# maybeLx/MVSFormerPlusPlus

Hardware: NVIDIA H100
Metric: depth-maps/sec (hot path: FMT + 4-stage cascade) (higher is better)
Workload: dtype f32

## Files before the change

mvsformerplusplus_b200/csrc/warp_corr.cu:

```cuda
#include <float.h>

#include <atomic>
#include <mutex>

#include "warp_geom.cuh"

namespace mvsf {

bool warp_tile_supported(const float* feat, int C, int G, int D, int H, int W);
int warp_tile_entropy(const float* feat, const float* homs, const float* depth, float* entropy, int V, int C, int D, int H,
                      int W, cudaStream_t s);
int warp_tile_aggregate(const float* feat, const float* homs, const float* depth, const float* vis, float* volume, int V, int C,
                        int D, int H, int W, cudaStream_t s);
bool warp_stream_store_supported(const float* feat, const float* corr, int C, int G, int D, int H, int W);
int warp_stream_entropy_store(const float* feat, const float* homs, const float* depth, float* entropy, float* corr, int V,
                              int H, int W, int* select, int max_miss_permille, cudaStream_t s);

constexpr int kMaxGenericD = 512;

template <int C>
struct WC {
  static constexpr int LPP = C / 4, P = 32 / LPP, DCH = 2 * LPP;
};
struct __align__(16) TapTable {
  int4 off[64];
  float4 wt[64];
};

template <int C>
__device__ __forceinline__ void build_taps(TapTable& tb, const float* __restrict__ depth, const Hom& m, const float3& ray,
                                           const CoordConst& cc, int p1, int d0, int D, int HW, int H, int W, int lane) {
  constexpr int P = WC<C>::P;
#pragma unroll
  for (int k = 0; k < 2; ++k) {
    const int t = lane + 32 * k;
    const int d = d0 + t / P;
    const float dv = (d < D) ? __ldg(depth + (size_t)d * HW + p1) : 1.0f;
    float ix, iy;
    warp_coord_fast(ray, m, dv, cc, ix, iy);
    int4 off;
    float4 wt;
    make_tap_fast(ix, iy, W, H, C, off, wt);
    tb.off[t] = off;
    tb.wt[t] = wt;
  }
}
__device__ __forceinline__ float4 gather4(const float* __restrict__ base, const int4& o, const float4& w) {
  float4 a = ldg4(base + o.x), b = ldg4(base + o.y), c = ldg4(base + o.z), d = ldg4(base + o.w);
  float4 s;
// ... 83 lines not shown
      }
    }
    __syncwarp();
    ReduceScatter<DCH, LPP>::run(part, lip);
#pragma unroll
    for (int i = 0; i < SPL; ++i) {
      const int d = d0 + lip * SPL + i;
      sims[ch * SPL + i] = (d < D) ? part[i] * gscale : -FLT_MAX;
    }
  }
  float mx = -FLT_MAX;
  for (int i = 0; i < nch * SPL; ++i) mx = fmaxf(mx, sims[i]);
#pragma unroll
  for (int o = LPP / 2; o > 0; o >>= 1) mx = fmaxf(mx, __shfl_xor_sync(0xffffffffu, mx, o));
  float Z = 0.f;
  for (int i = 0; i < nch * SPL; ++i) {
    sims[i] = (sims[i] == -FLT_MAX) ? 0.f : expf(sims[i] - mx);
    Z += sims[i];
  }
#pragma unroll
  for (int o = LPP / 2; o > 0; o >>= 1) Z += __shfl_xor_sync(0xffffffffu, Z, o);
  float ent = 0.f;
  for (int i = 0; i < nch * SPL; ++i) {
    float pr = __fdiv_rn(sims[i], Z);
    ent -= pr * logf(pr + 1e-7f);
  }
#pragma unroll
  for (int o = LPP / 2; o > 0; o >>= 1) ent += __shfl_xor_sync(0xffffffffu, ent, o);
  if (active && lip == 0) entropy[(size_t)v * HW + p2] = ent;
  if (STRIDED) __syncwarp();
  } while (STRIDED && (bx += (int)gridDim.x) * 8 * P < HW);
}

template <int C, int CPG>
__global__ void __launch_bounds__(256)
warp_corr_aggregate_kernel(const float* __restrict__ feat, const float* __restrict__ homs,
                           const float* __restrict__ depth, const float* __restrict__ vis,
                           float* __restrict__ volume, int V, int D, int H, int W) {
  constexpr int LPP = WC<C>::LPP, P = WC<C>::P, DCH = WC<C>::DCH;
  constexpr int G = C / CPG;
  constexpr int NGL = (CPG >= 4) ? 1 : 4 / CPG;
  constexpr int LPG = (CPG >= 4) ? CPG / 4 : 1;
  static_assert(LPG == 1 || LPG == 2, "C/G must be 1, 2, 4 or 8");
  __shared__ TapTable tables[8];
  const int lane = threadIdx.x & 31, warp = threadIdx.x >> 5;
  TapTable& tb = tables[warp];
  const int HW = H * W;
  const int pix0 = (blockIdx.x * 8 + warp) * P;
  if (pix0 >= HW) return;
  const int p1 = min(pix0 + lane % P, HW - 1);
  const int p2raw = pix0 + lane / LPP;
  const bool active = p2raw < HW;
  const int p2 = active ? p2raw : HW - 1;
  const int lip = lane % LPP, pi = lane / LPP;
  const CoordConst cc = make_coord_const(W, H);
  const int y1 = p1 / W, x1 = p1 - y1 * W;
  const float fx = (float)x1, fy = (float)y1;
  const float4 r = ldg4(feat + (size_t)p2 * C + lip * 4);
  constexpr float inv_cpg = 1.0f / (float)CPG;

  for (int d0 = 0; d0 < D; d0 += DCH) {
    float acc[NGL][DCH];
#pragma unroll
    for (int g = 0; g < NGL; ++g)
#pragma unroll
      for (int i = 0; i < DCH; ++i) acc[g][i] = 0.f;
    float wsum = 0.f;
    for (int v = 0; v < V - 1; ++v) {
      const Hom m = load_hom(homs + (size_t)v * 12);
      const float3 ray = ref_ray(m, fx, fy);
      build_taps<C>(tb, depth, m, ray, cc, p1, d0, D, HW, H, W, lane);
      __syncwarp();
      const float* __restrict__ src = feat + (size_t)(v + 1) * HW * C + lip * 4;
      const float w = __ldg(vis + (size_t)v * HW + p2);
      wsum = __fadd_rn(wsum, w);
#pragma unroll
      for (int di = 0; di < DCH; ++di) {
        const int4 o = tb.off[di * P + pi];
        const float4 wt = tb.wt[di * P + pi];
        const float4 s = gather4(src, o, wt);
        if (CPG >= 4) {
// ... 8 lines not shown
          acc[NGL > 2 ? 2 : 0][di] = fmaf(r.z * s.z, w, acc[NGL > 2 ? 2 : 0][di]);
          acc[NGL > 3 ? 3 : 0][di] = fmaf(r.w * s.w, w, acc[NGL > 3 ? 3 : 0][di]);
        }
      }
      __syncwarp();
    }
    const float den = __fadd_rn(wsum, 1e-6f);
    if (LPG == 2) {
      ReduceScatter<DCH, 2>::run(acc[0], lip & 1);
      if (active) {
        const int dbase = d0 + (lip & 1) * (DCH / 2);
#pragma unroll
        for (int i = 0; i < DCH / 2; ++i)
          if (dbase + i < D) volume[((size_t)(dbase + i) * HW + p2) * G + (lip >> 1)] = __fdiv_rn(acc[0][i], den);
      }
    } else if (active) {
#pragma unroll
      for (int di = 0; di < DCH; ++di) {
        if (d0 + di < D) {
          float* o = volume + ((size_t)(d0 + di) * HW + p2) * G;
          if (NGL == 1) {
            o[lip] = __fdiv_rn(acc[0][di], den);
          } else if (NGL == 2) {
            *reinterpret_cast<float2*>(o + lip * 2) = make_float2(__fdiv_rn(acc[0][di], den), __fdiv_rn(acc[NGL > 1 ? 1 : 0][di], den));
          } else {
            *reinterpret_cast<float4*>(o + lip * 4) =
                make_float4(__fdiv_rn(acc[0][di], den), __fdiv_rn(acc[NGL > 1 ? 1 : 0][di], den),
                            __fdiv_rn(acc[NGL > 2 ? 2 : 0][di], den), __fdiv_rn(acc[NGL > 3 ? 3 : 0][di], den));
          }
        }
      }
    }
  }
}

__global__ void homo_warp_kernel(const float* __restrict__ src, const float* __restrict__ hom,
                                 const float* __restrict__ depth, float* __restrict__ warped,
                                 uint8_t* __restrict__ mask, int C, int D, int H, int W) {
  const int HW = H * W;
  int p = blockIdx.x * blockDim.x + threadIdx.x;
  int d = blockIdx.y;
  if (p >= HW) return;
  int y = p / W, x = p - y * W;
  const Hom m = load_hom(hom);
  const float3 ray = ref_ray(m, (float)x, (float)y);
  const float half_w = (float)(W - 1) * 0.5f, half_h = (float)(H - 1) * 0.5f;
  float ix, iy, z;
  warp_coord(ray, m, __ldg(depth + (size_t)d * HW + p), half_w, half_h, (float)(W - 1), (float)(H - 1), ix, iy, z);
  Tap t = make_tap(ix, iy, W, H, C);
  for (int c = 0; c < C; ++c) {
    float a = __ldg(src + t.o00 + c), b = __ldg(src + t.o01 + c), cc = __ldg(src + t.o10 + c), dd = __ldg(src + t.o11 + c);
    warped[((size_t)c * D + d) * HW + p] = fmaf(dd, t.w11, fmaf(cc, t.w10, fmaf(b, t.w01, a * t.w00)));
  }
  if (mask) {
    bool out = (ix > (float)(W - 1)) || (ix < 0.0f) || (iy > (float)(H - 1)) || (iy < 0.0f) || (z <= 0.0f);
    mask[(size_t)d * HW + p] = out ? 1 : 0;
  }
}

template <int C>
static void launch_entropy(const float* feat, const float* homs, const float* depth, float* entropy, float* corr, int V, int G,
                           int D, int H, int W, cudaStream_t s) {
  constexpr int P = WC<C>::P;
  dim3 grid(cdiv((long long)H * W, 8 * P), V - 1);
  if (corr) {
    if (D == WC<C>::DCH)
      warp_corr_entropy_kernel<C, false, C / 8><<<grid, 256, 0, s>>>(feat, homs, depth, entropy, corr, G, D, H, W, nullptr);
    else
      warp_corr_entropy_kernel<C, true, C / 8><<<grid, 256, 0, s>>>(feat, homs, depth, entropy, corr, G, D, H, W, nullptr);
  } else if (D == WC<C>::DCH) {
    warp_corr_entropy_kernel<C, false, 0><<<grid, 256, 0, s>>>(feat, homs, depth, entropy, nullptr, G, D, H, W, nullptr);
  } else {
    warp_corr_entropy_kernel<C, true, 0><<<grid, 256, 0, s>>>(feat, homs, depth, entropy, nullptr, G, D, H, W, nullptr);
  }
}

static void launch_entropy_behind_select(const float* feat, const float* homs, const float* depth, float* entropy, float* corr,
                                         int V, int H, int W, cudaStream_t s, const int* skip_if) {
  constexpr int P = WC<8>::P;
  dim3 grid(cdiv((long long)H * W, 8 * P), V - 1);
  const int cap = device_sm_count(current_device()) * 16;
  if ((int)grid.x > cap) grid.x = cap;
  warp_corr_entropy_kernel<8, false, 1, true><<<grid, 256, 0, s>>>(feat, homs, depth, entropy, corr, 8, WC<8>::DCH, H, W, skip_if);
}

__global__ void __launch_bounds__(256)
corr_aggregate_kernel(const float* __restrict__ corr, const float* __restrict__ vis, float* __restrict__ volume, int V, int D,
                      int HW) {
  const size_t i = (size_t)blockIdx.x * blockDim.x + threadIdx.x;
  const size_t total = (size_t)D * HW * 2;
  if (i >= total) return;
  const size_t dp = i >> 1;
  const int p = (int)(dp % HW);
  float4 acc = make_float4(0.f, 0.f, 0.f, 0.f);
  float wsum = 0.f;
  for (int v = 0; v < V - 1; ++v) {
    const float w = __ldg(vis + (size_t)v * HW + p);
    const float4 c = ldg4(corr + ((size_t)v * D * HW + dp) * 8 + (i & 1) * 4);
    wsum = __fadd_rn(wsum, w);
    acc.x = fmaf(c.x, w, acc.x); acc.y = fmaf(c.y, w, acc.y); acc.z = fmaf(c.z, w, acc.z); acc.w = fmaf(c.w, w, acc.w);
  }
  const float den = __fadd_rn(wsum, 1e-6f);
  *reinterpret_cast<float4*>(volume + dp * 8 + (i & 1) * 4) =
      make_float4(__fdiv_rn(acc.x, den), __fdiv_rn(acc.y, den), __fdiv_rn(acc.z, den), __fdiv_rn(acc.w, den));
}

template <int C, int CPG>
static int launch_aggregate(const float* feat, const float* homs, const float* depth, const float* vis, float* volume,
                            int V, int D, int H, int W, cudaStream_t s) {
  constexpr int P = WC<C>::P;
  dim3 grid(cdiv((long long)H * W, 8 * P));
  warp_corr_aggregate_kernel<C, CPG><<<grid, 256, 0, s>>>(feat, homs, depth, vis, volume, V, D, H, W);
  return 0;
}

}

using namespace mvsf;

static int g_use_tile = 1;
constexpr int kMaxMissPermille = 60;

constexpr int kSelectSlots = 256;
static int* g_select[16] = {};
static std::atomic<unsigned> g_select_next{0};
static std::atomic<int*> g_select_last{nullptr};
static std::mutex g_select_mu;
static int* select_slot() {
  const int dev = current_device();
  if (dev < 0 || dev >= 16) return nullptr;
  if (!g_select[dev]) {
    std::lock_guard<std::mutex> lock(g_select_mu);
    if (!g_select[dev]) {
      int* p = nullptr;
      if (cudaMalloc(&p, sizeof(int) * 8 * kSelectSlots) != cudaSuccess) return nullptr;
      cudaMemset(p, 0, sizeof(int) * 8 * kSelectSlots);
      g_select[dev] = p;
    }
  }
  int* slot = g_select[dev] + 8 * (g_select_next.fetch_add(1) % kSelectSlots);
  g_select_last.store(slot);
  return slot;
}

extern "C" {
// ... 18 lines not shown
int mvsf_warp_corr_plan(int C, int G, int D, int H, int W, int V, size_t spill_budget_bytes) {
  if (G != 8 || !(C == 8 || C == 16 || C == 32 || C == 64)) return 1;
  const size_t spill = (size_t)4 * (size_t)(V > 1 ? V - 1 : 1) * G * D * H * W;
  return spill > spill_budget_bytes ? 1 : 0;
}
int mvsf_warp_corr_entropy(const float* feat, const float* homs, const float* depth, float* entropy, int V, int C,
                           int G, int D, int H, int W, mvsf_stream_t stream) {
  return warp_corr_entropy_impl(feat, homs, depth, entropy, nullptr, V, C, G, D, H, W, stream);
}

int mvsf_warp_corr_entropy_store(const float* feat, const float* homs, const float* depth, float* entropy, float* corr,
                                 int V, int C, int G, int D, int H, int W, mvsf_stream_t stream) {
  MVSF_REQUIRE(corr && ((uintptr_t)corr & 15) == 0 && G == 8, "warp_corr_entropy_store: corr must be 16-byte aligned and G == 8");
  return warp_corr_entropy_impl(feat, homs, depth, entropy, corr, V, C, G, D, H, W, stream);
}

int mvsf_corr_aggregate(const float* corr, const float* vis, float* volume, int V, int G, int D, int H, int W,
                        mvsf_stream_t stream) {
  MVSF_REQUIRE(corr && vis && volume && V >= 2 && G == 8 && D >= 1 && H > 0 && W > 0, "corr_aggregate: bad arguments (G must be 8)");
  const size_t total = (size_t)D * H * W * 2;
  corr_aggregate_kernel<<<cdiv((long long)total, 256), 256, 0, (cudaStream_t)stream>>>(corr, vis, volume, V, D, H * W);
  MVSF_LAUNCH_CHECK("corr_aggregate");
  return MVSF_OK;
}

static int warp_corr_entropy_impl(const float* feat, const float* homs, const float* depth, float* entropy, float* corr, int V,
                                  int C, int G, int D, int H, int W, mvsf_stream_t stream) {
  MVSF_REQUIRE(feat && homs && depth && entropy, "warp_corr_entropy: null pointer");
  MVSF_REQUIRE(V >= 2 && H > 0 && W > 0 && D >= 1, "warp_corr_entropy: bad shape");
  MVSF_REQUIRE(G <= C, "G must <= C!");
  MVSF_REQUIRE(C % G == 0 && (C == 8 || C == 16 || C == 32 || C == 64), "warp_corr_entropy: C must be 8/16/32/64, C %% G == 0");
  MVSF_REQUIRE(D <= kMaxGenericD, "warp_corr_entropy: D <= %d", kMaxGenericD);
  cudaStream_t s = (cudaStream_t)stream;
  const bool pipeline = corr && g_use_tile && warp_stream_store_supported(feat, corr, C, G, D, H, W);
  if (pipeline && g_use_tile == 2) {
    int rc = warp_stream_entropy_store(feat, homs, depth, entropy, corr, V, H, W, nullptr, kMaxMissPermille, s);
    if (rc) return rc;
    MVSF_LAUNCH_CHECK("warp_stream_entropy_store");
    return MVSF_OK;
  }
  int* select = pipeline ? select_slot() : nullptr;
  if (select) {
    int rc = warp_stream_entropy_store(feat, homs, depth, entropy, corr, V, H, W, select, kMaxMissPermille, s);
    if (rc) return rc;
    count_launch();
    MVSF_LAUNCH_CHECK("warp_stream_entropy_store");
    launch_entropy_behind_select(feat, homs, depth, entropy, corr, V, H, W, s, select);
    MVSF_LAUNCH_CHECK("warp_corr_entropy");
    return MVSF_OK;
  }
  if (!corr && g_use_tile && warp_tile_supported(feat, C, G, D, H, W)) {
    int rc = warp_tile_entropy(feat, homs, depth, entropy, V, C, D, H, W, s);
    if (rc) return rc;
    MVSF_LAUNCH_CHECK("warp_tile_entropy");
    return MVSF_OK;
  }
  switch (C) {
    case 8: launch_entropy<8>(feat, homs, depth, entropy, corr, V, G, D, H, W, s); break;
    case 16: launch_entropy<16>(feat, homs, depth, entropy, corr, V, G, D, H, W, s); break;
    case 32: launch_entropy<32>(feat, homs, depth, entropy, corr, V, G, D, H, W, s); break;
    default: launch_entropy<64>(feat, homs, depth, entropy, corr, V, G, D, H, W, s); break;
  }
  MVSF_LAUNCH_CHECK("warp_corr_entropy");
  return MVSF_OK;
}

int mvsf_warp_corr_aggregate(const float* feat, const float* homs, const float* depth, const float* vis,
                             float* volume, int V, int C, int G, int D, int H, int W, mvsf_stream_t stream) {
  MVSF_REQUIRE(feat && homs && depth && vis && volume, "warp_corr_aggregate: null pointer");
  MVSF_REQUIRE(V >= 2 && H > 0 && W > 0 && D >= 1, "warp_corr_aggregate: bad shape");
  MVSF_REQUIRE(G <= C, "G must <= C!");
  MVSF_REQUIRE(G == 8 && (C == 8 || C == 16 || C == 32 || C == 64), "warp_corr_aggregate: G must be 8 and C in 8/16/32/64");
  cudaStream_t s = (cudaStream_t)stream;
  if (g_use_tile && warp_tile_supported(feat, C, G, D, H, W)) {
    int rc = warp_tile_aggregate(feat, homs, depth, vis, volume, V, C, D, H, W, s);
    if (rc) return rc;
    MVSF_LAUNCH_CHECK("warp_tile_aggregate");
    return MVSF_OK;
  }
  switch (C) {
    case 8: launch_aggregate<8, 1>(feat, homs, depth, vis, volume, V, D, H, W, s); break;
    case 16: launch_aggregate<16, 2>(feat, homs, depth, vis, volume, V, D, H, W, s); break;
    case 32: launch_aggregate<32, 4>(feat, homs, depth, vis, volume, V, D, H, W, s); break;
    default: launch_aggregate<64, 8>(feat, homs, depth, vis, volume, V, D, H, W, s); break;
  }
  MVSF_LAUNCH_CHECK("warp_corr_aggregate");
  return MVSF_OK;
}

int mvsf_homo_warp(const float* src_nhwc, const float* hom, const float* depth, float* warped, uint8_t* mask, int C,
                   int D, int H, int W, mvsf_stream_t stream) {
  MVSF_REQUIRE(src_nhwc && hom && depth && warped && C > 0 && D > 0 && H > 0 && W > 0 && D <= 65535, "homo_warp: bad arguments");
  dim3 grid(cdiv(H * W, 128), D);
  homo_warp_kernel<<<grid, 128, 0, (cudaStream_t)stream>>>(src_nhwc, hom, depth, warped, mask, C, D, H, W);
  MVSF_LAUNCH_CHECK("homo_warp");
  return MVSF_OK;
}
}
```

mvsformerplusplus_b200/csrc/warp_tile.cu:

```cuda
#include <float.h>
#include <limits.h>

#include "warp_geom.cuh"
#include "wgmma.cuh"

namespace mvsf {
namespace wt {
using namespace gmma;

constexpr int TW = 32, THREADS = 256;
constexpr int kMaxD = 512;
constexpr int kPassBBlocks8 = 3;
constexpr int kPsBlocks = 2, kPsNbuf = 3;

template <int C>
struct Cfg {
  static constexpr int LPX = C / 8;
  static constexpr int PIX = THREADS / LPX;
  static constexpr int TROWS = PIX / TW;
  static constexpr int WX = 64, WY = 16;
  static constexpr int POS = 2 * C * 4;
  static constexpr int P = WX * POS;
  static constexpr uint32_t BYTES = (WY / 2) * P;
};

__device__ __forceinline__ void mbar_wait_warp(uint32_t bar, uint32_t parity) {
  if ((threadIdx.x & 31) == 0) {
    uint32_t it = 0;
    while (!mbar_try_wait(bar, parity))
      if (++it > (1u << MVSF_MBAR_SPIN_LOG2)) __trap();
  }
  __syncwarp();
}
__device__ __forceinline__ float4 lds128(uint32_t addr) {
  float4 v;
  asm volatile("ld.shared.v4.f32 {%0, %1, %2, %3}, [%4];" : "=f"(v.x), "=f"(v.y), "=f"(v.z), "=f"(v.w) : "r"(addr));
  return v;
}
__device__ __forceinline__ void fma4(float4& acc, float w, const float4& t) {
  acc = make_float4(fmaf(t.x, w, acc.x), fmaf(t.y, w, acc.y), fmaf(t.z, w, acc.z), fmaf(t.w, w, acc.w));
}
__device__ __forceinline__ float dot4(const float4& a, const float4& b) { return fmaf(a.w, b.w, fmaf(a.z, b.z, fmaf(a.y, b.y, a.x * b.x))); }

struct Lane {
  bool b0, b1, b2;
  uint32_t base[2];
};
template <int C>
__device__ __forceinline__ Lane make_lane(int lane, int sub, uint32_t win, int& chA, int& chB) {
  Lane L;
  if (C == 8) {
    L.b0 = lane & 1; L.b1 = (lane >> 1) & 1; L.b2 = (lane >> 2) & 1;
    L.base[0] = win + (L.b0 ? 16 : 0);
    L.base[1] = win + (L.b0 ? 0 : 16);
    chA = L.b0 ? 4 : 0; chB = L.b0 ? 0 : 4;
  } else {
    L.b0 = false; L.b1 = (lane >> 1) & 1; L.b2 = (lane >> 2) & 1;
    const int q0 = 2 * sub + (L.b1 ? 1 : 0), q1 = 2 * sub + (L.b1 ? 0 : 1);
    L.base[0] = win + q0 * 16;
    L.base[1] = win + q1 * 16;
    chA = q0 * 4; chB = q1 * 4;
  }
  return L;
}

template <int C>
__device__ __forceinline__ void gather_window(const Lane& L, int lx, int ly, float fx, float fy, float4& sA, float4& sB) {
  using K = Cfg<C>;
  const float gx = 1.0f - fx, gy = 1.0f - fy;
  const bool yodd = ly & 1;
// ... 243 lines not shown
      for (int k = 0; k < DCHT; ++k) accA[k] = accB[k] = make_float4(0.f, 0.f, 0.f, 0.f);
      for (int v = 0; v < V - 1; ++v) {
        const ViewCtx<C> vc = make_view(v);
        const float w = __ldg(vis + (size_t)v * HW + p);
        process_chunk<C, DCHT>(&map, sh, win, slot, phase, L, vc, v + 1, depth_p, HW, d0, n, active, cc, W, H,
                               [&](int k, const float4& sA, const float4& sB) {
                                 accA[k].x = fmaf(qA.x * sA.x, w, accA[k].x); accA[k].y = fmaf(qA.y * sA.y, w, accA[k].y);
                                 accA[k].z = fmaf(qA.z * sA.z, w, accA[k].z); accA[k].w = fmaf(qA.w * sA.w, w, accA[k].w);
                                 accB[k].x = fmaf(qB.x * sB.x, w, accB[k].x); accB[k].y = fmaf(qB.y * sB.y, w, accB[k].y);
                                 accB[k].z = fmaf(qB.z * sB.z, w, accB[k].z); accB[k].w = fmaf(qB.w * sB.w, w, accB[k].w);
                               });
      }
      if (active) {
#pragma unroll
        for (int k = 0; k < DCHT; ++k) {
          if (k < n) {
            float* o = out + ((size_t)(d0 + k) * HW + p) * 8;
            if (C == 8) {
              *reinterpret_cast<float4*>(o + chA) = make_float4(__fdiv_rn(accA[k].x, den), __fdiv_rn(accA[k].y, den),
                                                                __fdiv_rn(accA[k].z, den), __fdiv_rn(accA[k].w, den));
              *reinterpret_cast<float4*>(o + chB) = make_float4(__fdiv_rn(accB[k].x, den), __fdiv_rn(accB[k].y, den),
                                                                __fdiv_rn(accB[k].z, den), __fdiv_rn(accB[k].w, den));
            } else {
              *reinterpret_cast<float2*>(o + chA / 2) = make_float2(__fdiv_rn(accA[k].x + accA[k].y, den), __fdiv_rn(accA[k].z + accA[k].w, den));
              *reinterpret_cast<float2*>(o + chB / 2) = make_float2(__fdiv_rn(accB[k].x + accB[k].y, den), __fdiv_rn(accB[k].z + accB[k].w, den));
            }
          }
        }
      }
    }
  }
}

template <int C>
struct PsCfg {
  static constexpr int NCONS = 256 * Cfg<C>::LPX;
  static constexpr int THREADS = NCONS + 32;
  static constexpr int TROWS = 8;
};

template <int NBUF>
struct PsShared {
  unsigned long long full[NBUF], empty[NBUF];
  int origin[NBUF][2];
};

template <int C>
__device__ __forceinline__ int2 sample_pixel(int tile, int tiles_x, int lane, int W, int H) {
  const int sr = (lane >> 3) * 2 + 1, sc = (lane & 7) * 4 + 1;
  return make_int2(min((tile % tiles_x) * TW + sc, W - 1), min((tile / tiles_x) * PsCfg<C>::TROWS + sr, H - 1));
}
template <int C>
__device__ __forceinline__ int2 predict_window(const Hom& m, const float3& ray, float d_first, float d_last, const CoordConst& cc,
                                               int W, int H) {
  Bbox b;
#pragma unroll
  for (int e = 0; e < 2; ++e) {
    float ix, iy;
    warp_coord_lean(ray, m, e ? d_last : d_first, cc, ix, iy);
    b.add(split_coord(ix, iy, W, H));
  }
  b.reduce_warp();
  return window_origin<C>(b);
}

template <int C, int D, int NBUF>
__global__ void __launch_bounds__(PsCfg<C>::THREADS, kPsBlocks)
warp_stream_entropy_store_kernel(const __grid_constant__ CUtensorMap map, const float* __restrict__ feat,
                                 const float* __restrict__ homs, const float* __restrict__ depth, float* __restrict__ entropy,
                                 float* __restrict__ corr, int V, int H, int W, int tiles_x, int ntiles,
                                 const int* __restrict__ select) {
  using K = Cfg<C>;
  using P = PsCfg<C>;
  extern __shared__ __align__(128) unsigned char smem_raw[];
  __shared__ PsShared<NBUF> sh;
  if (select && *select == 0) return;
  const uint32_t win0 = (smem_u32(smem_raw) + 127u) & ~127u;
  const int tid = threadIdx.x, lane = tid & 31, warp = tid >> 5;
  const int HW = H * W;
  if (tid == 0) {
    for (int b = 0; b < NBUF; ++b) { mbar_init(smem_u32(&sh.full[b]), 1); mbar_init(smem_u32(&sh.empty[b]), P::NCONS / 32); }
    fence_barrier_init();
  }
  __syncthreads();
  const CoordConst cc = make_coord_const(W, H);
  const int my_tiles = (ntiles - (int)blockIdx.x + (int)gridDim.x - 1) / (int)gridDim.x;

  if (warp == P::NCONS / 32) {
    int j = 0;
    for (int t = 0; t < my_tiles; ++t) {
      const int2 sp = sample_pixel<C>((int)blockIdx.x + t * (int)gridDim.x, tiles_x, lane, W, H);
      const int p = sp.y * W + sp.x;
      const float d_first = __ldg(depth + p), d_last = __ldg(depth + (size_t)(D - 1) * HW + p);
      for (int v = 0; v < V - 1; ++v, ++j) {
        const int buf = j % NBUF;
        const Hom m = load_hom(homs + (size_t)v * 12);
        const int2 o = predict_window<C>(m, ref_ray(m, (float)sp.x, (float)sp.y), d_first, d_last, cc, W, H);
        mbar_wait_warp(smem_u32(&sh.empty[buf]), (uint32_t)(((j / NBUF) & 1) ^ 1));
        if (lane == 0) {
          sh.origin[buf][0] = o.x;
          sh.origin[buf][1] = o.y;
          const uint32_t bar = smem_u32(&sh.full[buf]);
          expect_tx(bar, K::BYTES);
          tma_load_5d(win0 + (uint32_t)buf * K::BYTES, &map, 0, 0, o.x, o.y >> 1, v + 1, bar);
        }
        __syncwarp();
      }
    }
    return;
  }

  const int pix_in_cta = tid / K::LPX, sub = tid % K::LPX;
  int chA, chB;
  const Lane L0 = make_lane<C>(lane, sub, 0u, chA, chB);
  constexpr float inv_cpg = 8.0f / (float)C;
  int j = 0;
  for (int t = 0; t < my_tiles; ++t) {
    const int tile = (int)blockIdx.x + t * (int)gridDim.x;
    const int px = (tile % tiles_x) * TW + (pix_in_cta % TW), py = (tile / tiles_x) * P::TROWS + (pix_in_cta / TW);
    const bool active = (px < W) && (py < H);
    const int p = min(py, H - 1) * W + min(px, W - 1);
    const float fxp = (float)min(px, W - 1), fyp = (float)min(py, H - 1);
    const float4 rA = ldg4(feat + (size_t)p * C + chA), rB = ldg4(feat + (size_t)p * C + chB);
    float dv[D];
#pragma unroll
    for (int k = 0; k < D; ++k) dv[k] = __ldg(depth + (size_t)k * HW + p);
    for (int v = 0; v < V - 1; ++v, ++j) {
      const int buf = j % NBUF;
      const Hom m = load_hom(homs + (size_t)v * 12);
      const float3 ray = ref_ray(m, fxp, fyp);
      const float* __restrict__ src = feat + (size_t)(v + 1) * HW * C;
      mbar_wait_warp(smem_u32(&sh.full[buf]), (uint32_t)((j / NBUF) & 1));
      const int ox = sh.origin[buf][0], oy = sh.origin[buf][1];
      const uint32_t wbuf = win0 + (uint32_t)buf * K::BYTES;
      const Lane L = {L0.b0, L0.b1, L0.b2, {wbuf + L0.base[0], wbuf + L0.base[1]}};
      float sims[D];
      float mx = -FLT_MAX;
#pragma unroll
      for (int k = 0; k < D; ++k) {
        float ix, iy;
        warp_coord_lean(ray, m, dv[k], cc, ix, iy);
        TapCoord tc = split_coord(ix, iy, W, H);
        tc.inb = tc.inb && active;
        float4 sA = make_float4(0.f, 0.f, 0.f, 0.f), sB = sA;
        const int lx = tc.x0 - ox, ly = tc.y0 - oy;
        const bool inwin = in_window<C>(tc.inb, lx, ly);
        gather_window<C>(L, inwin ? lx : 0, inwin ? ly : 0, tc.fx, tc.fy, sA, sB);
        if (!inwin) {
          sA = make_float4(0.f, 0.f, 0.f, 0.f); sB = sA;
          if (tc.inb) gather_global<C>(src + chA, src + chB, ix, iy, W, H, sA, sB);
        }
        if (active) {
          float* cp = corr + (((size_t)v * D + k) * HW + p) * 8;
          if (C == 8) {
            *reinterpret_cast<float4*>(cp + chA) = make_float4(rA.x * sA.x, rA.y * sA.y, rA.z * sA.z, rA.w * sA.w);
            *reinterpret_cast<float4*>(cp + chB) = make_float4(rB.x * sB.x, rB.y * sB.y, rB.z * sB.z, rB.w * sB.w);
          } else {
            *reinterpret_cast<float2*>(cp + chA / 2) = make_float2(fmaf(rA.y, sA.y, rA.x * sA.x) * inv_cpg, fmaf(rA.w, sA.w, rA.z * sA.z) * inv_cpg);
            *reinterpret_cast<float2*>(cp + chB / 2) = make_float2(fmaf(rB.y, sB.y, rB.x * sB.x) * inv_cpg, fmaf(rB.w, sB.w, rB.z * sB.z) * inv_cpg);
          }
        }
        float s = dot4(rA, sA) + dot4(rB, sB);
        if (K::LPX == 2) s += __shfl_xor_sync(0xffffffffu, s, 1);
        s *= inv_cpg;
        sims[k] = s;
        mx = fmaxf(mx, s);
      }
      __syncwarp();
      if (lane == 0) mbar_arrive(smem_u32(&sh.empty[buf]));
      float Z = 0.f, ent = 0.f;
#pragma unroll
      for (int k = 0; k < D; ++k) { sims[k] = __expf(sims[k] - mx); Z += sims[k]; }
      const float rZ = __fdiv_rn(1.0f, Z);
#pragma unroll
      for (int k = 0; k < D; ++k) { const float pr = sims[k] * rZ; ent -= pr * __logf(pr + 1e-7f); }
      if (active && sub == 0) entropy[(size_t)v * HW + p] = ent;
    }
  }
}


template <int C, int D>
__global__ void __launch_bounds__(1024)
warp_stream_select_kernel(const float* __restrict__ homs, const float* __restrict__ depth, int V, int H, int W, int tiles_x,
                          int ntiles, int max_miss_permille, int* __restrict__ select) {
  const int lane = threadIdx.x & 31, HW = H * W;
  const CoordConst cc = make_coord_const(W, H);
  const int2 sp = sample_pixel<C>((int)(((long long)blockIdx.x * ntiles) / gridDim.x), tiles_x, lane, W, H);
  const int p = sp.y * W + sp.x;
  float dv[D];
#pragma unroll
  for (int k = 0; k < D; ++k) dv[k] = __ldg(depth + (size_t)k * HW + p);
  unsigned int tot = 0u, miss = 0u;
  for (int v = threadIdx.x >> 5; v < V - 1; v += blockDim.x >> 5) {
    const Hom m = load_hom(homs + (size_t)v * 12);
    const float3 ray = ref_ray(m, (float)sp.x, (float)sp.y);
    const int2 o = predict_window<C>(m, ray, dv[0], dv[D - 1], cc, W, H);
#pragma unroll
    for (int k = 0; k < D; ++k) {
      float ix, iy;
      warp_coord_lean(ray, m, dv[k], cc, ix, iy);
      const TapCoord tc = split_coord(ix, iy, W, H);
      if (!tc.inb) continue;
      ++tot;
      if (!in_window<C>(true, tc.x0 - o.x, tc.y0 - o.y)) ++miss;
    }
  }
  tot = __reduce_add_sync(0xffffffffu, tot);
  miss = __reduce_add_sync(0xffffffffu, miss);
// ... 35 lines not shown
  using K = Cfg<C>;
  auto kern = warp_tile_kernel<C, MODE, DCHT, GENERIC>;
  static DeviceOnce once;
  const int dev = current_device();
  const size_t smem = K::BYTES + 128;
  if (once.need(dev)) {
    MVSF_CUDA_OK(cudaFuncSetAttribute(kern, cudaFuncAttributeMaxDynamicSharedMemorySize, (int)smem));
    once.done(dev);
  }
  CUtensorMap map;
  int rc = make_window_map<C>(&map, feat, V, H, W);
  if (rc) return rc;
  dim3 grid(cdiv(W, TW), cdiv(H, K::TROWS));
  kern<<<grid, THREADS, smem, s>>>(map, feat, homs, depth, vis, out, V, D, H, W, dch);
  return MVSF_OK;
}

template <int C>
static int dispatch(int mode, const float* feat, const float* homs, const float* depth, const float* vis, float* out, int V,
                    int D, int H, int W, cudaStream_t s) {
  if (mode == 0) {
    if (D <= 4) return launch<C, 0, 4, false>(feat, homs, depth, vis, out, V, D, H, W, D, s);
    if (D <= 8) return launch<C, 0, 8, false>(feat, homs, depth, vis, out, V, D, H, W, D, s);
    int c = D / 24;
    c = c < 2 ? 2 : (c > 8 ? 8 : c);
    return launch<C, 0, 8, true>(feat, homs, depth, vis, out, V, D, H, W, c, s);
  }
  if (D <= 4) return launch<C, 1, 4, false>(feat, homs, depth, vis, out, V, D, H, W, D, s);
  int c = D <= 8 ? D : D / 24;
  c = c < 2 ? 2 : (c > 8 ? 8 : c);
  return launch<C, 1, 8, false>(feat, homs, depth, vis, out, V, D, H, W, c, s);
}

template <int C, int D, int NBUF>
static int launch_stream_store(const float* feat, const float* homs, const float* depth, float* entropy, float* corr, int V,
                               int H, int W, int* select, int max_miss_permille, cudaStream_t s) {
  using K = Cfg<C>;
  auto kern = warp_stream_entropy_store_kernel<C, D, NBUF>;
  static DeviceOnce once;
  const int dev = current_device();
  const size_t smem = (size_t)NBUF * K::BYTES + 128;
  if (once.need(dev)) {
    MVSF_CUDA_OK(cudaFuncSetAttribute(kern, cudaFuncAttributeMaxDynamicSharedMemorySize, (int)smem));
    once.done(dev);
  }
  CUtensorMap map;
  int rc = make_window_map<C>(&map, feat, V, H, W);
  if (rc) return rc;
  const int tiles_x = cdiv(W, TW), tiles_y = cdiv(H, PsCfg<C>::TROWS), ntiles = tiles_x * tiles_y;
  const int cap = device_sm_count(dev) * kPsBlocks;
  if (select) {
    const int nsample = ntiles < 96 ? ntiles : 96, warps = V - 1 < 32 ? V - 1 : 32;
    warp_stream_select_kernel<C, D><<<nsample, 32 * warps, 0, s>>>(homs, depth, V, H, W, tiles_x, ntiles, max_miss_permille, select);
  }
  kern<<<ntiles < cap ? ntiles : cap, PsCfg<C>::THREADS, smem, s>>>(map, feat, homs, depth, entropy, corr, V, H, W, tiles_x, ntiles, select);
  return MVSF_OK;
}

}

bool warp_tile_supported(const float* feat, int C, int G, int D, int H, int W) {
  return (C == 8 || C == 16) && G == 8 && (H % 2 == 0) && H >= 2 && W >= 2 && D >= 1 && D <= wt::kMaxD &&
         ((uintptr_t)feat & 15) == 0 && ((long long)W * C * 4) % 16 == 0;
}
int warp_tile_entropy(const float* feat, const float* homs, const float* depth, float* entropy, int V, int C, int D, int H,
                      int W, cudaStream_t s) {
  return C == 8 ? wt::dispatch<8>(0, feat, homs, depth, nullptr, entropy, V, D, H, W, s)
                : wt::dispatch<16>(0, feat, homs, depth, nullptr, entropy, V, D, H, W, s);
}
int warp_tile_aggregate(const float* feat, const float* homs, const float* depth, const float* vis, float* volume, int V, int C,
                        int D, int H, int W, cudaStream_t s) {
  return C == 8 ? wt::dispatch<8>(1, feat, homs, depth, vis, volume, V, D, H, W, s)
                : wt::dispatch<16>(1, feat, homs, depth, vis, volume, V, D, H, W, s);
}

bool warp_stream_store_supported(const float* feat, const float* corr, int C, int G, int D, int H, int W) {
  return warp_tile_supported(feat, C, G, D, H, W) && C == 8 && D == 4 && ((uintptr_t)corr & 15) == 0;
}
int warp_stream_entropy_store(const float* feat, const float* homs, const float* depth, float* entropy, float* corr, int V,
                              int H, int W, int* select, int max_miss_permille, cudaStream_t s) {
  return wt::launch_stream_store<8, 4, wt::kPsNbuf>(feat, homs, depth, entropy, corr, V, H, W, select, max_miss_permille, s);
}

}
```

mvsformerplusplus_b200/hotpath.py:

```python
import math

import torch
import torch.nn as nn

from . import _lib, packing
from .config import load_args, stage_list, validate_args
from .params import build_fmt, build_fpn_decoder, build_fpn_encoder, build_stage, build_vit, build_vit_decoder


def _f32c(t):
    if t.dtype != torch.float32:
        t = t.float()
    return t if t.is_contiguous() else t.contiguous()


def _require_cuda(t, what):
    if not t.is_cuda:
        raise RuntimeError(f"{what}: expected a CUDA tensor (the hot path has no CPU fallback)")


def to_nhwc(x):
    n, c, h, w = x.shape
    xp = x.permute(0, 2, 3, 1)
    if x.dtype == torch.float32 and xp.is_contiguous():
# ... 99 lines not shown
            if (tuple(cfg["down_rate"]) != (2, 4, 4) or cfg["mid_channel"] != 64 or cfg["num_heads"] != 4
                    or cfg["mlp_ratio"] != 4):
                raise NotImplementedError("transformer regulariser: only the shipped geometry (down_rate (2,4,4), "
                                          "mid 64, 4 heads, mlp_ratio 4) is implemented")
            gemm, small = packing.pack_costreg_tr(sd, "cost_reg.", cfg["layer_num"])
            pk.update(kind="tr", layers=cfg["layer_num"], tc=split_weights_f16(gemm.to(device)))
        else:
            kind, conv, small = packing.pack_costreg_unet(sd, "cost_reg.")
            pk.update(kind=kind, tc=pack_unet_tc(kind, conv.to(device)))
        pk["w"] = small.to(device)
        return pk

    def _softmax_scale(self, n_tokens):
        tc = self.args["transformer_config"][self.stage_idx]
        scale = (tc["mid_channel"] // tc["num_heads"]) ** -0.5
        if tc.get("softmax_scale", None) is not None:
            scale *= math.log(n_tokens, tc["train_avg_length"])
        return scale

    def _forward_one(self, feat_nhwc, proj, depth_values, tmp, position3d, pk, keep=False):
        V, H, W, C = feat_nhwc.shape
        D = depth_values.shape[0]
        dev = feat_nhwc.device
        G = stage_list(self.args["base_ch"], self.stage_idx)
        if G > C:
            raise AssertionError("G must <= C!")
        f32 = dict(device=dev, dtype=torch.float32)
        homs = torch.empty((V - 1) * 12, **f32)
        kinv = torch.empty(9, **f32)
        _lib.call("mvsf_compose_geometry", proj, V, homs, kinv)
        entropy = torch.empty((V - 1, H, W), **f32)
        vis = torch.empty((V - 1, H, W), **f32)
        volume = torch.empty((D, H, W, G), **f32)
        two_gathers = _lib.lib().mvsf_warp_corr_plan(C, G, D, H, W, V, self.corr_spill_budget_bytes) == 1
        if not two_gathers:
            corr = torch.empty((V - 1, D, H, W, G), **f32)
            _lib.call("mvsf_warp_corr_entropy_store", feat_nhwc, homs, depth_values, entropy, corr, V, C, G, D, H, W)
            _lib.call("mvsf_vis_cnn", entropy, pk["vis"], vis, V - 1, H, W)
            _lib.call("mvsf_corr_aggregate", corr, vis, volume, V, G, D, H, W)
            del corr
        else:
            _lib.call("mvsf_warp_corr_entropy", feat_nhwc, homs, depth_values, entropy, V, C, G, D, H, W)
            _lib.call("mvsf_vis_cnn", entropy, pk["vis"], vis, V - 1, H, W)
            _lib.call("mvsf_warp_corr_aggregate", feat_nhwc, homs, depth_values, vis, volume, V, C, G, D, H, W)
        kept = dict(entropy=entropy, vis_weight=vis, volume_mean=volume.clone() if keep else None) if keep else None
        logits = torch.empty((D, H, W), **f32)
        if pk["kind"] == "tr":
            ws = _lib.workspace("mvsf_costreg_tr_workspace_bytes", G, D, H, W, device=dev)
            n_tok = (D // 2) * (H // 4) * (W // 4)
            _lib.call("mvsf_costreg_tr_forward", volume, position3d, pk["w"], pk["tc"], pk["tc"].numel() // 2, logits,
                      ws, ws.numel() * 4, G, D, H, W, pk["layers"], float(self._softmax_scale(n_tok)))
        else:
            ws = _lib.workspace("mvsf_costreg_unet_workspace_bytes", pk["kind"], G, D, H, W, device=dev)
            _lib.call("mvsf_costreg_unet_forward", pk["kind"], volume, pk["w"], pk["tc"], logits, ws, ws.numel() * 4,
                      G, D, H, W)
        prob = torch.empty((D, H, W), **f32)
        depth = torch.empty((H, W), **f32)
        conf = torch.empty((H, W), **f32)
        _lib.call("mvsf_softargmax", logits, depth_values, float(tmp), prob, depth, conf, D, H, W)
        return depth, prob, conf, logits, kept

    @torch.no_grad()
    def forward(self, features, proj_matrices, depth_values, tmp, position3d=None, keep_intermediates=False):
        if self.training:
            raise NotImplementedError("the hot path implements the eval-mode forward (test.py); call .eval()")
        if self.depth_type != "ce":
            raise NotImplementedError("depth_type must be 'ce'")
# ... 493 lines not shown
```

Measured before the change: 51.16.

## Use TMA stream kernel for entropy and aggregation, avoid corr spill at C8/D4

Generalizes the TMA-pipelined stream kernel into store, entropy-only and aggregate modes. The aggregate mode accumulates visibility-weighted correlations in shared memory and writes the normalized volume directly. The final stage (C==8, D==4) is forced onto the two-gather path so the corr tensor is never written and re-read. Also adds a strided, skip-if fallback aggregate kernel behind the selector, and narrows tile support for C=16 to D>8. The cost is a second warp/gather pass plus extra shared memory for accumulators.

```diff
diff --git a/mvsformerplusplus_b200/csrc/warp_corr.cu b/mvsformerplusplus_b200/csrc/warp_corr.cu
--- a/mvsformerplusplus_b200/csrc/warp_corr.cu
+++ b/mvsformerplusplus_b200/csrc/warp_corr.cu
@@ -12,9 +12,10 @@
                       int W, cudaStream_t s);
 int warp_tile_aggregate(const float* feat, const float* homs, const float* depth, const float* vis, float* volume, int V, int C,
                         int D, int H, int W, cudaStream_t s);
-bool warp_stream_store_supported(const float* feat, const float* corr, int C, int G, int D, int H, int W);
-int warp_stream_entropy_store(const float* feat, const float* homs, const float* depth, float* entropy, float* corr, int V,
-                              int H, int W, int* select, int max_miss_permille, cudaStream_t s);
+bool warp_stream_supported(const float* feat, const float* out, int C, int G, int D, int H, int W);
+int warp_stream(int mode, const float* feat, const float* homs, const float* depth, const float* vis, float* entropy, float* out,
+                int V, int H, int W, int* select, int max_miss_permille, cudaStream_t s);
+constexpr int kStreamStore = 0, kStreamEntropy = 1, kStreamAggregate = 2;
 
 constexpr int kMaxGenericD = 512;
 
@@ -164,21 +165,24 @@
   } while (STRIDED && (bx += (int)gridDim.x) * 8 * P < HW);
 }
 
-template <int C, int CPG>
-__global__ void __launch_bounds__(256)
+template <int C, int CPG, bool STRIDED = false>
+__global__ void __launch_bounds__(256, STRIDED ? 4 : 0)
 warp_corr_aggregate_kernel(const float* __restrict__ feat, const float* __restrict__ homs,
                            const float* __restrict__ depth, const float* __restrict__ vis,
-                           float* __restrict__ volume, int V, int D, int H, int W) {
+                           float* __restrict__ volume, int V, int D, int H, int W, const int* __restrict__ skip_if) {
   constexpr int LPP = WC<C>::LPP, P = WC<C>::P, DCH = WC<C>::DCH;
   constexpr int G = C / CPG;
   constexpr int NGL = (CPG >= 4) ? 1 : 4 / CPG;
   constexpr int LPG = (CPG >= 4) ? CPG / 4 : 1;
   static_assert(LPG == 1 || LPG == 2, "C/G must be 1, 2, 4 or 8");
+  if (skip_if && *skip_if != 0) return;
   __shared__ TapTable tables[8];
   const int lane = threadIdx.x & 31, warp = threadIdx.x >> 5;
   TapTable& tb = tables[warp];
   const int HW = H * W;
-  const int pix0 = (blockIdx.x * 8 + warp) * P;
+  int bx = blockIdx.x;
+  do {
+  const int pix0 = (bx * 8 + warp) * P;
   if (pix0 >= HW) return;
   const int p1 = min(pix0 + lane % P, HW - 1);
   const int p2raw = pix0 + lane / LPP;
@@ -253,6 +257,7 @@
       }
     }
   }
+  } while (STRIDED && (bx += (int)gridDim.x) * 8 * P < HW);
 }
 
 __global__ void homo_warp_kernel(const float* __restrict__ src, const float* __restrict__ hom,
@@ -296,13 +301,22 @@
   }
 }
 
+static int behind_select_blocks(int H, int W) {
+  const int blocks = (int)cdiv((long long)H * W, 8 * WC<8>::P), cap = device_sm_count(current_device()) * 16;
+  return blocks < cap ? blocks : cap;
+}
 static void launch_entropy_behind_select(const float* feat, const float* homs, const float* depth, float* entropy, float* corr,
                                          int V, int H, int W, cudaStream_t s, const int* skip_if) {
-  constexpr int P = WC<8>::P;
-  dim3 grid(cdiv((long long)H * W, 8 * P), V - 1);
-  const int cap = device_sm_count(current_device()) * 16;
-  if ((int)grid.x > cap) grid.x = cap;
-  warp_corr_entropy_kernel<8, false, 1, true><<<grid, 256, 0, s>>>(feat, homs, depth, entropy, corr, 8, WC<8>::DCH, H, W, skip_if);
+  const dim3 grid(behind_select_blocks(H, W), V - 1);
+  if (corr)
+    warp_corr_entropy_kernel<8, false, 1, true><<<grid, 256, 0, s>>>(feat, homs, depth, entropy, corr, 8, WC<8>::DCH, H, W, skip_if);
+  else
+    warp_corr_entropy_kernel<8, false, 0, true><<<grid, 256, 0, s>>>(feat, homs, depth, entropy, nullptr, 8, WC<8>::DCH, H, W, skip_if);
+}
+static void launch_aggregate_behind_select(const float* feat, const float* homs, const float* depth, const float* vis,
+                                           float* volume, int V, int H, int W, cudaStream_t s, const int* skip_if) {
+  warp_corr_aggregate_kernel<8, 1, true><<<behind_select_blocks(H, W), 256, 0, s>>>(feat, homs, depth, vis, volume, V,
+                                                                                    WC<8>::DCH, H, W, skip_if);
 }
 
 __global__ void __launch_bounds__(256)
@@ -331,7 +345,7 @@
                             int V, int D, int H, int W, cudaStream_t s) {
   constexpr int P = WC<C>::P;
   dim3 grid(cdiv((long long)H * W, 8 * P));
-  warp_corr_aggregate_kernel<C, CPG><<<grid, 256, 0, s>>>(feat, homs, depth, vis, volume, V, D, H, W);
+  warp_corr_aggregate_kernel<C, CPG><<<grid, 256, 0, s>>>(feat, homs, depth, vis, volume, V, D, H, W, nullptr);
   return 0;
 }
 
@@ -416,19 +430,20 @@
   MVSF_REQUIRE(C % G == 0 && (C == 8 || C == 16 || C == 32 || C == 64), "warp_corr_entropy: C must be 8/16/32/64, C %% G == 0");
   MVSF_REQUIRE(D <= kMaxGenericD, "warp_corr_entropy: D <= %d", kMaxGenericD);
   cudaStream_t s = (cudaStream_t)stream;
-  const bool pipeline = corr && g_use_tile && warp_stream_store_supported(feat, corr, C, G, D, H, W);
+  const int mode = corr ? kStreamStore : kStreamEntropy;
+  const bool pipeline = g_use_tile && warp_stream_supported(feat, corr, C, G, D, H, W);
   if (pipeline && g_use_tile == 2) {
-    int rc = warp_stream_entropy_store(feat, homs, depth, entropy, corr, V, H, W, nullptr, kMaxMissPermille, s);
+    int rc = warp_stream(mode, feat, homs, depth, nullptr, entropy, corr, V, H, W, nullptr, kMaxMissPermille, s);
     if (rc) return rc;
-    MVSF_LAUNCH_CHECK("warp_stream_entropy_store");
+    MVSF_LAUNCH_CHECK("warp_stream");
     return MVSF_OK;
   }
   int* select = pipeline ? select_slot() : nullptr;
   if (select) {
-    int rc = warp_stream_entropy_store(feat, homs, depth, entropy, corr, V, H, W, select, kMaxMissPermille, s);
+    int rc = warp_stream(mode, feat, homs, depth, nullptr, entropy, corr, V, H, W, select, kMaxMissPermille, s);
     if (rc) return rc;
     count_launch();
-    MVSF_LAUNCH_CHECK("warp_stream_entropy_store");
+    MVSF_LAUNCH_CHECK("warp_stream");
     launch_entropy_behind_select(feat, homs, depth, entropy, corr, V, H, W, s, select);
     MVSF_LAUNCH_CHECK("warp_corr_entropy");
     return MVSF_OK;
@@ -456,6 +471,23 @@
   MVSF_REQUIRE(G <= C, "G must <= C!");
   MVSF_REQUIRE(G == 8 && (C == 8 || C == 16 || C == 32 || C == 64), "warp_corr_aggregate: G must be 8 and C in 8/16/32/64");
   cudaStream_t s = (cudaStream_t)stream;
+  const bool pipeline = g_use_tile && warp_stream_supported(feat, volume, C, G, D, H, W);
+  if (pipeline && g_use_tile == 2) {
+    int rc = warp_stream(kStreamAggregate, feat, homs, depth, vis, nullptr, volume, V, H, W, nullptr, kMaxMissPermille, s);
+    if (rc) return rc;
+    MVSF_LAUNCH_CHECK("warp_stream");
+    return MVSF_OK;
+  }
+  int* select = pipeline ? select_slot() : nullptr;
+  if (select) {
+    int rc = warp_stream(kStreamAggregate, feat, homs, depth, vis, nullptr, volume, V, H, W, select, kMaxMissPermille, s);
+    if (rc) return rc;
+    count_launch();
+    MVSF_LAUNCH_CHECK("warp_stream");
+    launch_aggregate_behind_select(feat, homs, depth, vis, volume, V, H, W, s, select);
+    MVSF_LAUNCH_CHECK("warp_corr_aggregate");
+    return MVSF_OK;
+  }
   if (g_use_tile && warp_tile_supported(feat, C, G, D, H, W)) {
     int rc = warp_tile_aggregate(feat, homs, depth, vis, volume, V, C, D, H, W, s);
     if (rc) return rc;
diff --git a/mvsformerplusplus_b200/csrc/warp_tile.cu b/mvsformerplusplus_b200/csrc/warp_tile.cu
--- a/mvsformerplusplus_b200/csrc/warp_tile.cu
+++ b/mvsformerplusplus_b200/csrc/warp_tile.cu
@@ -36,6 +36,9 @@
   float4 v;
   asm volatile("ld.shared.v4.f32 {%0, %1, %2, %3}, [%4];" : "=f"(v.x), "=f"(v.y), "=f"(v.z), "=f"(v.w) : "r"(addr));
   return v;
+}
+__device__ __forceinline__ void sts128(uint32_t addr, const float4& v) {
+  asm volatile("st.shared.v4.f32 [%0], {%1, %2, %3, %4};" :: "r"(addr), "f"(v.x), "f"(v.y), "f"(v.z), "f"(v.w));
 }
 __device__ __forceinline__ void fma4(float4& acc, float w, const float4& t) {
   acc = make_float4(fmaf(t.x, w, acc.x), fmaf(t.y, w, acc.y), fmaf(t.z, w, acc.z), fmaf(t.w, w, acc.w));
@@ -345,6 +348,8 @@
   }
 }
 
+enum PsMode { kPsStore = 0, kPsEntropy = 1, kPsAggregate = 2 };
+
 template <int C>
 struct PsCfg {
   static constexpr int NCONS = 256 * Cfg<C>::LPX;
@@ -377,14 +382,19 @@
   return window_origin<C>(b);
 }
 
-template <int C, int D, int NBUF>
+constexpr int kPsAggNbuf = 2;
+template <int C, int D>
+struct PsAcc {
+  static constexpr uint32_t BYTES = (uint32_t)D * 2 * PsCfg<C>::NCONS * 16;
+};
+template <int C, int D, int NBUF, int MODE>
 __global__ void __launch_bounds__(PsCfg<C>::THREADS, kPsBlocks)
-warp_stream_entropy_store_kernel(const __grid_constant__ CUtensorMap map, const float* __restrict__ feat,
-                                 const float* __restrict__ homs, const float* __restrict__ depth, float* __restrict__ entropy,
-                                 float* __restrict__ corr, int V, int H, int W, int tiles_x, int ntiles,
-                                 const int* __restrict__ select) {
+warp_stream_kernel(const __grid_constant__ CUtensorMap map, const float* __restrict__ feat, const float* __restrict__ homs,
+                   const float* __restrict__ depth, const float* __restrict__ vis, float* __restrict__ entropy,
+                   float* __restrict__ out, int V, int H, int W, int tiles_x, int ntiles, const int* __restrict__ select) {
   using K = Cfg<C>;
   using P = PsCfg<C>;
+  static_assert(MODE != kPsAggregate || C == 8, "the aggregation epilogue is written for C == G == 8");
   extern __shared__ __align__(128) unsigned char smem_raw[];
   __shared__ PsShared<NBUF> sh;
   if (select && *select == 0) return;
@@ -438,11 +448,23 @@
     float dv[D];
 #pragma unroll
     for (int k = 0; k < D; ++k) dv[k] = __ldg(depth + (size_t)k * HW + p);
+    const uint32_t acc_s = win0 + (uint32_t)NBUF * K::BYTES + (uint32_t)tid * 16u;
+    constexpr uint32_t kQuad = 16u * P::NCONS;
+    if (MODE == kPsAggregate) {
+#pragma unroll
+      for (int k = 0; k < 2 * D; ++k) sts128(acc_s + k * kQuad, make_float4(0.f, 0.f, 0.f, 0.f));
+    }
+    float wsum = 0.f;
     for (int v = 0; v < V - 1; ++v, ++j) {
       const int buf = j % NBUF;
       const Hom m = load_hom(homs + (size_t)v * 12);
       const float3 ray = ref_ray(m, fxp, fyp);
       const float* __restrict__ src = feat + (size_t)(v + 1) * HW * C;
+      float w = 0.f;
+      if (MODE == kPsAggregate) {
+        w = __ldg(vis + (size_t)v * HW + p);
+        wsum = __fadd_rn(wsum, w);
+      }
       mbar_wait_warp(smem_u32(&sh.full[buf]), (uint32_t)((j / NBUF) & 1));
       const int ox = sh.origin[buf][0], oy = sh.origin[buf][1];
       const uint32_t wbuf = win0 + (uint32_t)buf * K::BYTES;
@@ -463,8 +485,16 @@
           sA = make_float4(0.f, 0.f, 0.f, 0.f); sB = sA;
           if (tc.inb) gather_global<C>(src + chA, src + chB, ix, iy, W, H, sA, sB);
         }
-        if (active) {
-          float* cp = corr + (((size_t)v * D + k) * HW + p) * 8;
+        if (MODE == kPsAggregate) {
+          const float4 a = lds128(acc_s + 2 * k * kQuad), b = lds128(acc_s + (2 * k + 1) * kQuad);
+          sts128(acc_s + 2 * k * kQuad, make_float4(fmaf(rA.x * sA.x, w, a.x), fmaf(rA.y * sA.y, w, a.y),
+                                                    fmaf(rA.z * sA.z, w, a.z), fmaf(rA.w * sA.w, w, a.w)));
+          sts128(acc_s + (2 * k + 1) * kQuad, make_float4(fmaf(rB.x * sB.x, w, b.x), fmaf(rB.y * sB.y, w, b.y),
+                                                          fmaf(rB.z * sB.z, w, b.z), fmaf(rB.w * sB.w, w, b.w)));
+          continue;
+        }
+        if (MODE == kPsStore && active) {
+          float* cp = out + (((size_t)v * D + k) * HW + p) * 8;
           if (C == 8) {
             *reinterpret_cast<float4*>(cp + chA) = make_float4(rA.x * sA.x, rA.y * sA.y, rA.z * sA.z, rA.w * sA.w);
             *reinterpret_cast<float4*>(cp + chB) = make_float4(rB.x * sB.x, rB.y * sB.y, rB.z * sB.z, rB.w * sB.w);
@@ -481,6 +511,7 @@
       }
       __syncwarp();
       if (lane == 0) mbar_arrive(smem_u32(&sh.empty[buf]));
+      if (MODE == kPsAggregate) continue;
       float Z = 0.f, ent = 0.f;
 #pragma unroll
       for (int k = 0; k < D; ++k) { sims[k] = __expf(sims[k] - mx); Z += sims[k]; }
@@ -488,6 +519,16 @@
 #pragma unroll
       for (int k = 0; k < D; ++k) { const float pr = sims[k] * rZ; ent -= pr * __logf(pr + 1e-7f); }
       if (active && sub == 0) entropy[(size_t)v * HW + p] = ent;
+    }
+    if (MODE == kPsAggregate && active) {
+      const float den = __fadd_rn(wsum, 1e-6f);
+#pragma unroll
+      for (int k = 0; k < D; ++k) {
+        float* o = out + ((size_t)k * HW + p) * 8;
+        const float4 a = lds128(acc_s + 2 * k * kQuad), b = lds128(acc_s + (2 * k + 1) * kQuad);
+        *reinterpret_cast<float4*>(o + chA) = make_float4(__fdiv_rn(a.x, den), __fdiv_rn(a.y, den), __fdiv_rn(a.z, den), __fdiv_rn(a.w, den));
+        *reinterpret_cast<float4*>(o + chB) = make_float4(__fdiv_rn(b.x, den), __fdiv_rn(b.y, den), __fdiv_rn(b.z, den), __fdiv_rn(b.w, den));
+      }
     }
   }
 }
@@ -589,14 +630,14 @@
   return launch<C, 1, 8, false>(feat, homs, depth, vis, out, V, D, H, W, c, s);
 }
 
-template <int C, int D, int NBUF>
-static int launch_stream_store(const float* feat, const float* homs, const float* depth, float* entropy, float* corr, int V,
-                               int H, int W, int* select, int max_miss_permille, cudaStream_t s) {
-  using K = Cfg<C>;
-  auto kern = warp_stream_entropy_store_kernel<C, D, NBUF>;
+template <int C, int D, int NBUF, int MODE>
+static int launch_stream(const float* feat, const float* homs, const float* depth, const float* vis, float* entropy, float* out,
+                         int V, int H, int W, int* select, int max_miss_permille, cudaStream_t s) {
+  using K = Cfg<C>;
+  auto kern = warp_stream_kernel<C, D, NBUF, MODE>;
   static DeviceOnce once;
   const int dev = current_device();
-  const size_t smem = (size_t)NBUF * K::BYTES + 128;
+  const size_t smem = (size_t)NBUF * K::BYTES + 128 + (MODE == kPsAggregate ? PsAcc<C, D>::BYTES : 0);
   if (once.need(dev)) {
     MVSF_CUDA_OK(cudaFuncSetAttribute(kern, cudaFuncAttributeMaxDynamicSharedMemorySize, (int)smem));
     once.done(dev);
@@ -610,14 +651,15 @@
     const int nsample = ntiles < 96 ? ntiles : 96, warps = V - 1 < 32 ? V - 1 : 32;
     warp_stream_select_kernel<C, D><<<nsample, 32 * warps, 0, s>>>(homs, depth, V, H, W, tiles_x, ntiles, max_miss_permille, select);
   }
-  kern<<<ntiles < cap ? ntiles : cap, PsCfg<C>::THREADS, smem, s>>>(map, feat, homs, depth, entropy, corr, V, H, W, tiles_x, ntiles, select);
+  kern<<<ntiles < cap ? ntiles : cap, PsCfg<C>::THREADS, smem, s>>>(map, feat, homs, depth, vis, entropy, out, V, H, W, tiles_x,
+                                                                      ntiles, select);
   return MVSF_OK;
 }
 
 }
 
 bool warp_tile_supported(const float* feat, int C, int G, int D, int H, int W) {
-  return (C == 8 || C == 16) && G == 8 && (H % 2 == 0) && H >= 2 && W >= 2 && D >= 1 && D <= wt::kMaxD &&
+  return (C == 8 || (C == 16 && D > 8)) && G == 8 && (H % 2 == 0) && H >= 2 && W >= 2 && D >= 1 && D <= wt::kMaxD &&
          ((uintptr_t)feat & 15) == 0 && ((long long)W * C * 4) % 16 == 0;
 }
 int warp_tile_entropy(const float* feat, const float* homs, const float* depth, float* entropy, int V, int C, int D, int H,
@@ -631,12 +673,17 @@
                 : wt::dispatch<16>(1, feat, homs, depth, vis, volume, V, D, H, W, s);
 }
 
-bool warp_stream_store_supported(const float* feat, const float* corr, int C, int G, int D, int H, int W) {
-  return warp_tile_supported(feat, C, G, D, H, W) && C == 8 && D == 4 && ((uintptr_t)corr & 15) == 0;
-}
-int warp_stream_entropy_store(const float* feat, const float* homs, const float* depth, float* entropy, float* corr, int V,
-                              int H, int W, int* select, int max_miss_permille, cudaStream_t s) {
-  return wt::launch_stream_store<8, 4, wt::kPsNbuf>(feat, homs, depth, entropy, corr, V, H, W, select, max_miss_permille, s);
-}
-
-}
+bool warp_stream_supported(const float* feat, const float* out, int C, int G, int D, int H, int W) {
+  return warp_tile_supported(feat, C, G, D, H, W) && C == 8 && D == 4 && ((uintptr_t)out & 15) == 0;
+}
+int warp_stream(int mode, const float* feat, const float* homs, const float* depth, const float* vis, float* entropy, float* out,
+                int V, int H, int W, int* select, int max_miss_permille, cudaStream_t s) {
+  using namespace wt;
+  switch (mode) {
+    case kPsStore: return launch_stream<8, 4, kPsNbuf, kPsStore>(feat, homs, depth, nullptr, entropy, out, V, H, W, select, max_miss_permille, s);
+    case kPsEntropy: return launch_stream<8, 4, kPsNbuf, kPsEntropy>(feat, homs, depth, nullptr, entropy, nullptr, V, H, W, select, max_miss_permille, s);
+    default: return launch_stream<8, 4, kPsAggNbuf, kPsAggregate>(feat, homs, depth, vis, nullptr, out, V, H, W, select, max_miss_permille, s);
+  }
+}
+
+}
diff --git a/mvsformerplusplus_b200/hotpath.py b/mvsformerplusplus_b200/hotpath.py
--- a/mvsformerplusplus_b200/hotpath.py
+++ b/mvsformerplusplus_b200/hotpath.py
@@ -155,7 +155,7 @@
         entropy = torch.empty((V - 1, H, W), **f32)
         vis = torch.empty((V - 1, H, W), **f32)
         volume = torch.empty((D, H, W, G), **f32)
-        two_gathers = _lib.lib().mvsf_warp_corr_plan(C, G, D, H, W, V, self.corr_spill_budget_bytes) == 1
+        two_gathers = (C == 8 and D == 4) or _lib.lib().mvsf_warp_corr_plan(C, G, D, H, W, V, self.corr_spill_budget_bytes) == 1
         if not two_gathers:
             corr = torch.empty((V - 1, D, H, W, G), **f32)
             _lib.call("mvsf_warp_corr_entropy_store", feat_nhwc, homs, depth_values, entropy, corr, V, C, G, D, H, W)
```

Result: faster. 52.22 (median of 6 runs) (+2.1%).
